# arkworks-rs/gemini

Measured on AMD Instinct MI355X. Metric: BLS12-381 G1 MSM throughput, higher is better.
Workload: dtype u32x12 Montgomery Fq (381-bit integer), u32x8 Fr; 1 GPU; 2^20 G1 MSM per GPU (BASELINE configs[1]: 2^20 G1 MSM on one MI355X); pairs_per_gpu=1048576

## Files before the change

### gemini_amd/capi.py

```python
from __future__ import annotations

import ctypes as C
import os

import numpy as np

_HERE = os.path.dirname(os.path.abspath(__file__))
LIB_PATH = os.environ.get("GM_LIB_PATH") or os.path.join(_HERE, "libgemini_hip.so")

GM_OK = 0
ERRORS = {-1: "GM_EINVAL", -2: "GM_ENOTINIT", -3: "GM_EHANDLE", -4: "GM_EHIP", -5: "GM_ENOMEM", -6: "GM_ESTATE"}

SYMBOLS = [
    "gm_init", "gm_shutdown", "gm_last_error", "gm_abi_version",
    "gm_g1_msm", "gm_g1_bases_register", "gm_g1_bases_free", "gm_g1_bases_len", "gm_g1_bases_download", "gm_g1_bases_precompute", "gm_set_auto_tables", "gm_g1_bases_table_info", "gm_pool_trim", "gm_g1_release_spare_tables", "gm_mem_stats", "gm_mem_reset_peak", "gm_runtime_info", "gm_snark_footprint", "gm_psnark_footprint", "gm_footprint_admit",
    "gm_g1_msm_h", "gm_g1_msm_v", "gm_g1_msm_v_batch", "gm_g1_msm_v_batch_partial", "gm_g1_msm_v_batch_at", "gm_g1_msm_d", "gm_g1_msm_d_partial", "gm_g1_sum",
    "gm_g1_msm_stream_new", "gm_g1_msm_stream_new_h", "gm_g1_msm_stream_add", "gm_g1_msm_stream_finalize", "gm_g1_msm_stream_free", "gm_host_alloc", "gm_host_free",
    "gm_g1_fixed_base_register", "gm_g1_srs_register", "gm_g1_srs_register_segments", "gm_set_msm_window", "gm_set_msm_table_min", "gm_set_msm_affine_levels", "gm_set_msm_split", "gm_set_msm_glv", "gm_prof_enable", "gm_prof_read", "gm_prof_read_clock",
    "gm_idx_register", "gm_idx_free", "gm_idx_len", "gm_idx_download", "gm_idx_extend_frequency", "gm_fr_gather", "gm_fr_alg_hash", "gm_fr_plookup_set", "gm_fr_add_scalar", "gm_fr_shift_monic",
    "gm_fr_acc_product", "gm_fr_tensor_range", "gm_fr_tensor_gather", "gm_fr_powers_gather", "gm_fr_alg_hash_from", "gm_fr_powers_range", "gm_fr_plookup_set_block", "gm_fr_shift_block", "gm_fr_product", "gm_fr_acc_product_block",
    "gm_sc_set_shard_rounds", "gm_sc_round_begin_many", "gm_psnark_shard_block", "gm_psnark_shard_level", "gm_psnark_shard_footprint", "gm_psnark_shard_key_new", "gm_psnark_index_sharded", "gm_psnark_new_time_sharded", "gm_snark_new_elastic_sharded",
    "gm_fr_vec_alloc", "gm_fr_vec_free", "gm_fr_vec_len", "gm_fr_vec_upload", "gm_fr_vec_download",
    "gm_fr_vec_fill", "gm_fr_vec_ptr", "gm_fr_vec_set_len",
    "gm_fr_reverse", "gm_fr_stride", "gm_fr_fold", "gm_fr_fold_chain", "gm_fr_powers", "gm_fr_tensor", "gm_fr_hadamard", "gm_fr_ip", "gm_fr_eval_le", "gm_fr_eval_le_batch",
    "gm_fr_lincomb", "gm_fr_scale_into", "gm_fr_scale_into_many", "gm_fr_add_at", "gm_fr_div_vanishing",
    "gm_spm_register", "gm_spm_free", "gm_spm_mul", "gm_spm_shape", "gm_snark_new_time", "gm_snark_new_elastic", "gm_psnark_new_time", "gm_psnark_new_elastic", "gm_psnark_preprocess", "gm_psnark_preprocess_free", "gm_psnark_index", "gm_spm_download",
    "gm_sc_new", "gm_sc_new_v", "gm_sc_new_borrow", "gm_sc_round", "gm_sc_round_begin", "gm_sc_round_end", "gm_sc_fold", "gm_sc_rounds", "gm_sc_final", "gm_sc_free",
    "gm_sc_set_shard", "gm_sc_lens", "gm_sc_download",
    "gm_sp_new", "gm_sp_new_v", "gm_sp_new_borrow", "gm_sp_round", "gm_sp_fold", "gm_sp_rounds", "gm_sp_final", "gm_sp_to_time", "gm_sp_free",
    "gm_sc_set_herring", "gm_hg1_new", "gm_hg1_round", "gm_hg1_fold", "gm_hg1_rounds", "gm_hg1_final", "gm_hg1_free",
    "gm_g2_msm", "gm_g2_bases_register", "gm_g2_bases_free", "gm_g2_bases_len", "gm_g2_bases_download", "gm_g2_msm_h", "gm_g2_msm_v", "gm_g2_msm_d", "gm_g2_sum",
    "gm_hg2_new", "gm_hg2_round", "gm_hg2_fold", "gm_hg2_rounds", "gm_hg2_final", "gm_hg2_free",
    "gm_pairing_multi", "gm_pairing_multi_h", "gm_gt_mul", "gm_gt_pow", "gm_gt_one", "gm_gt_final_exp",
# ... 121 lines not shown
```

### gemini_amd/csrc/capi.hip

```cpp
#include <cstring>
#include <vector>

#include "ctx.hpp"
#include "host_field.hpp"

namespace gm {

static thread_local char g_err[512] = "";
void set_error(const char* fmt, ...) {
  va_list ap;
  va_start(ap, fmt);
  vsnprintf(g_err, sizeof g_err, fmt, ap);
  va_end(ap);
}
int hip_fail(hipError_t e, const char* what, const char* file, int line) {
  set_error("HIP error %d (%s) in %s at %s:%d", (int)e, hipGetErrorString(e), what, file, line);
  return e == hipErrorOutOfMemory ? GM_ENOMEM : GM_EHIP;
}

MemStats& mem_stats() {
  static MemStats* m = new MemStats;
  return *m;
}
void MemStats::note_cached(ptrdiff_t delta) {
// ... 665 lines not shown
  GM_CTX();
  GM_CHECK(c == 0 || (c >= 2 && c <= 22), GM_EINVAL, "gm_set_msm_window: c = %d not in {0} u [2, 22]", c);
  C->msm_c_override = c;
  return GM_OK;
}

int gm_set_msm_glv(int on) {
  GM_CTX();
#ifndef GM_EXPERIMENTS
  GM_CHECK(on == 0, GM_EINVAL, "gm_set_msm_glv: the GLV experiment is not in this build (make EXTRA=-DGM_EXPERIMENTS; DESIGN.md section 8)");
#endif
  C->msm_glv = on != 0;
  return GM_OK;
}

int gm_set_msm_split(int on) {
  GM_CTX();
#ifndef GM_EXPERIMENTS
  GM_CHECK(on == 0, GM_EINVAL, "gm_set_msm_split: the window-group experiment is not in this build (make EXTRA=-DGM_EXPERIMENTS; DESIGN.md section 8)");
#endif
  C->msm_split = on != 0;
  return GM_OK;
}

int gm_set_msm_affine_levels(int levels) {
  GM_CTX();
  GM_CHECK(levels >= -1 && levels <= 8, GM_EINVAL, "gm_set_msm_affine_levels: %d not in [-1, 8]", levels);
#ifndef GM_EXPERIMENTS
  if (levels == -1) levels = 0;
  GM_CHECK(levels == 0, GM_EINVAL, "gm_set_msm_affine_levels: the affine-level experiment is not in this build (make EXTRA=-DGM_EXPERIMENTS; DESIGN.md section 8)");
// ... 1443 lines not shown
```

### gemini_amd/csrc/ctx.hpp

```cpp
#pragma once
#include <hip/hip_runtime.h>

#include <atomic>
#include <cstdarg>
#include <cstdint>
#include <cstdio>
#include <map>
#include <memory>
#include <mutex>
#include <string>
#include <unordered_map>
#include <vector>

#include "../../include/gemini_hip.h"

namespace gmh {
struct Fq12;
}

namespace gm {

void set_error(const char* fmt, ...);
int hip_fail(hipError_t e, const char* what, const char* file, int line);

// ... 148 lines not shown
};
struct G2Workspace {
  DevBuf buckets, part, red[2], longs;
  uint64_t* host_out = nullptr;
  size_t host_out_cap = 0;
};

struct PairingWorkspace {
  DevBuf part[2];
  uint64_t* host_out = nullptr;
  DevBuf seg_tab;
  uint64_t* host_seg = nullptr;
  size_t host_seg_cap = 0;
};
struct MsmWorkspace;
struct MsmPending {
  MsmWorkspace* ws = nullptr;
  int slot = 0;
  bool empty = true;
  int Wb = 0, c = 0, m = 0;
  uint32_t nbits = 0, wf[3] = {0, 0, 0};
  size_t plane_off[3] = {0, 0, 0};
  size_t plane_count = 0;
  int multi_levels = 0;
  int multi_W = 0;
};
struct MsmStreamSlot {
  uint8_t *raw = nullptr, *packed = nullptr, *scalars = nullptr;
  size_t raw_cap = 0, packed_cap = 0, scalars_cap = 0;
  hipEvent_t copied;
  bool have_ev = false;
  bool inflight = false;
  MsmPending P;
};
struct MsmStream {
  std::mutex mu;
  size_t chunk = 0, stride = 96;
  int mont = 0;
  uint64_t bases_handle = 0;
  int64_t base0 = 0, next_base = 0, step = 1;
// ... 89 lines not shown
  hipStream_t part_tail[2 + MSM_SMALL_LANES] = {};
  hipEvent_t start_ev;
  bool have_start_ev = false;
  DevBuf fr_scratch;
  uint64_t* host_small = nullptr;
  uint8_t* sc_desc_host = nullptr;
  uint8_t* sc_desc_dev = nullptr;
  hipEvent_t sc_desc_copied[SC_DESC_SLOTS] = {};
  unsigned sc_desc_next = 0;
  uint64_t* host_batch = nullptr;
  size_t host_batch_cap = 0;
  int msm_c_override = 0;
  int msm_glv = 0;
  int msm_split = 0;
  int msm_affine_levels = 0;
  size_t msm_table_min = (size_t)1 << 17;
  int zero_copy = 3;
  std::atomic<int> msm_busy{0};
  bool auto_tables = true;
  size_t auto_tables_max = 0;
  int cu_count = 256;
};

Context* context();
struct MemStats {
  std::mutex mu;
  std::unordered_map<void*, size_t> sizes;
  size_t live = 0, peak_live = 0;
  size_t cached = 0;
  size_t peak_in_use = 0;
// ... 122 lines not shown
```

### gemini_amd/csrc/msm.hip

```cpp
#include <algorithm>
#include <atomic>
#include <chrono>
#include <condition_variable>
#include <cstdlib>
#include <cstring>
#include <functional>
#include <sched.h>
#include <cstdio>
#include <thread>
#include <vector>

#include "ctx.hpp"
#include "g1.cuh"
#include "host_field.hpp"

namespace gm {

constexpr uint32_t KEY_INV = 0xffffffffu;
constexpr int XYZZ_BYTES = 192;
constexpr int AFF_BYTES = 96;

struct DigitIter {
  uint32_t s[8];
  uint32_t carry;
// ... 298 lines not shown
    const bool live = e[w] != ~0ull;
    const uint32_t g = (uint32_t)(e[w] >> 32) >> sg.FB;
    const uint32_t r = wave_atomic_inc(cnt, live ? g : KEY_INV);
    if (live) buf[lst[g] + r] = e[w];
  }
  __syncthreads();
  for (uint32_t j = tid; j < m; j += 1024) {
    const uint64_t v = buf[j];
    const uint32_t g = (uint32_t)(v >> 32) >> sg.FB;
    tmp[base[g] + (j - lst[g])] = v;
  }
}

__global__ __launch_bounds__(1024) void k_sort1_scan(const uint32_t* __restrict__ gcount, uint32_t G,
                                                     uint32_t* __restrict__ goff, uint32_t* __restrict__ gcursor,
                                                     uint32_t* __restrict__ blkoff) {
  __shared__ uint32_t a[1024], b[1024];
  const uint32_t tid = threadIdx.x;
  const uint32_t per = (G + 1023u) / 1024u;
  uint32_t v[4], nb[4], sa = 0, sb = 0;
  for (uint32_t k = 0; k < per; k++) {
    const uint32_t g = tid * per + k;
    v[k] = g < G ? gcount[g] : 0u;
    nb[k] = (v[k] + SORT_CH - 1u) / SORT_CH;
    sa += v[k];
    sb += nb[k];
  }
  a[tid] = sa;
  b[tid] = sb;
  __syncthreads();
  for (uint32_t d = 1; d < 1024; d <<= 1) {
// ... 5 lines not shown
  }
  uint32_t ra = a[tid] - sa, rb = b[tid] - sb;
  for (uint32_t k = 0; k < per; k++) {
    const uint32_t g = tid * per + k;
    if (g < G) {
      goff[g] = ra;
      gcursor[g] = ra;
      blkoff[g] = rb;
    }
    ra += v[k];
    rb += nb[k];
  }
  if (tid == 1023) {
    goff[G] = a[1023];
    blkoff[G] = b[1023];
  }
}

template <bool SCATTER>
__global__ __launch_bounds__(256) void k_sort2(const uint64_t* __restrict__ tmp, const uint32_t* __restrict__ goff,
                                               const uint32_t* __restrict__ blkoff, SortGeom sg,
                                               uint32_t* __restrict__ counts_or_cursor, uint64_t* __restrict__ entries) {
  __shared__ uint32_t cnt[SORT_FMAX];
  __shared__ uint32_t base[SCATTER ? SORT_FMAX : 1];
  __shared__ uint32_t s_g;
  const uint32_t nf = 1u << sg.FB;
  if (blockIdx.x >= blkoff[sg.G]) return;
  if (threadIdx.x == 0) {
    uint32_t lo = 0, hi = sg.G;
    while (hi - lo > 1) {
// ... 100 lines not shown
  __syncthreads();
  for (uint32_t f = tid; f < nf; f += 1024) cnt[f] = 0;
  __syncthreads();
#pragma unroll
  for (uint32_t k = 0; k < PER; k++) {
    const uint32_t i = tid + k * 1024;
    const uint32_t f = (uint32_t)(e[k] >> 32) & mask;
    const uint32_t r = wave_atomic_inc(cnt, i < m ? f : KEY_INV);
    if (i < m) buf[lst[f] + r] = e[k];
  }
  __syncthreads();
  for (uint32_t i = tid; i < m; i += 1024) {
    const uint64_t v = buf[i];
    const uint32_t f = (uint32_t)(v >> 32) & mask;
    entries[base[f] + (i - lst[f])] = v;
  }
}

constexpr uint32_t SCAN_PER_THREAD = 16;
constexpr uint32_t SCAN_PER_BLOCK = 256 * SCAN_PER_THREAD;

GM_DEV uint32_t block_exclusive_scan_256(uint32_t v, uint32_t* lds , uint32_t* total) {
  const uint32_t tid = threadIdx.x;
  lds[tid] = v;
  __syncthreads();
  for (uint32_t d = 1; d < 256; d <<= 1) {
    uint32_t x = tid >= d ? lds[tid - d] : 0;
    __syncthreads();
    lds[tid] += x;
    __syncthreads();
// ... 523 lines not shown
  uint32_t n_out;
  uint32_t per_win;
  uint32_t win_stride;
  uint32_t n_lo, s_hi, s_lo, s_e, len;
  uint32_t nb;
  uint32_t lpo_shift;
  int out_canonical;
  const uint32_t* in_cnt;
};
struct GroupSumJobs {
  GroupSumArgs j[3];
  uint32_t blk_end[3];
  const uint32_t* err_src;
  uint32_t* err_dst;
  const unsigned long long* clk_src;
};

__global__ __launch_bounds__(256) void k_group_sum(GroupSumJobs J) {
  if (J.err_dst && blockIdx.x == 0 && threadIdx.x == 0) {
    *J.err_dst = *J.err_src;
    if (J.clk_src) {
      unsigned long long* d = reinterpret_cast<unsigned long long*>(J.err_dst + 2);
      d[0] = J.clk_src[0];
      d[1] = J.clk_src[1];
    }
  }
  const int job = blockIdx.x < J.blk_end[0] ? 0 : (blockIdx.x < J.blk_end[1] ? 1 : 2);
  const GroupSumArgs& a = J.j[job];
  const uint32_t blk0 = job == 0 ? 0u : J.blk_end[job - 1];
  const uint8_t* __restrict__ in = a.in;
  uint8_t* __restrict__ out = a.out;
  const uint32_t gt = (blockIdx.x - blk0) * blockDim.x + threadIdx.x;
  const uint32_t lpo = 1u << a.lpo_shift;
  const uint32_t o = gt >> a.lpo_shift, q = gt & (lpo - 1u);
  Acc30 acc;
// ... 628 lines not shown
  }
  if (batch_trace)
    fprintf(stderr, "[gm msm batch] %zu calls: %.3f ms, of which enqueueing %.3f ms, final drains %.3f ms\n", k,
            std::chrono::duration<double, std::milli>(std::chrono::steady_clock::now() - t_batch0).count(), enqueue_s * 1e3,
            std::chrono::duration<double, std::milli>(std::chrono::steady_clock::now() - t_enqueued).count());
  return GM_OK;
}

static int msm_enqueue(Context* C, MsmWorkspace& ws, MsmStreams sts, const Bases* bases, int64_t first, int64_t step, const void* d_scalars,
                       int mont, size_t n, int slot, MsmPending* P, int part, int nparts, const MsmMulti* multi) {
  hipStream_t st = sts.sort;
  const size_t nbases = bases->n;
  P->ws = &ws;
  P->slot = slot;
  P->multi_levels = 0;
  if (multi) {
    GM_CHECK(multi->levels >= 1 && multi->levels <= MULTI_MAX_LEVELS && nparts == 1, GM_EINVAL, "msm: %d fused calls (1 .. %d)", multi->levels, MULTI_MAX_LEVELS);
    GM_CHECK(nbases <= ((size_t)1 << 30), GM_EINVAL, "msm: a key of %zu points is too long for a fused pass (2^30)", nbases);
    n = 0;
    for (int l = 0; l < multi->levels; l++) {
      GM_CHECK(multi->n[l] >= 1 && multi->n[l] <= (multi->block ? MSM_MULTI_BLOCK_MAX_N : MSM_MULTI_MAX_N), GM_EINVAL, "msm: a fused call of %zu pairs", multi->n[l]);
      const int64_t lo = multi->start[l], hi = multi->start[l] + step * (int64_t)(multi->n[l] - 1);
      GM_CHECK(lo >= 0 && hi >= 0 && (size_t)lo < nbases && (size_t)hi < nbases, GM_EINVAL, "msm: base range [%lld .. %lld] outside registered bases (len %zu)",
               (long long)lo, (long long)hi, nbases);
      n += multi->n[l];
    }
    first = 0;
  }
  P->empty = n == 0;
  if (n == 0) return GM_OK;
// ... 78 lines not shown
  uint64_t Nacc = N;
  for (int l = 0; l < levels; l++) Nacc = Nacc / 2 + 2 * nbuckets + 2;

  static const int L_env = getenv("GM_MSM_L") ? atoi(getenv("GM_MSM_L")) : 0;
  const uint64_t Nacc_all = nparts > 1 ? Nall : Nacc;
  const uint64_t lanes0 = Nacc_all >= ((uint64_t)1 << 24) ? 262144 : 131072;
  static const uint64_t L_cap = getenv("GM_MSM_LCAP") ? (uint64_t)atoi(getenv("GM_MSM_LCAP")) : 256;
  uint32_t L = (uint32_t)std::min<uint64_t>(L_cap, std::max<uint64_t>(4, (Nacc_all + lanes0 - 1) / lanes0));
  if (L_env > 0) L = (uint32_t)L_env;
  L = (L + 1u) & ~1u;
  const uint64_t T0 = (Nacc + L - 1) / L;
  const uint64_t T0pad = (T0 + 255) / 256 * 256;
  const uint64_t E1 = 2 * T0pad;

  int rc;
  const size_t counts_words = (nbuckets + 2 + SORT_GMAX + 1 + 63) / 64 * 64;
  if ((rc = ws.counts.ensure(counts_words * 4))) return rc;
  if ((rc = ws.offsets.ensure((nbuckets + 1) * 4))) return rc;
  if ((rc = ws.cursor.ensure((nbuckets + 1) * 4))) return rc;
  if ((rc = ws.misc.ensure((nbuckets / SCAN_PER_BLOCK + 2) * 4))) return rc;
  if ((rc = ws.entries.ensure(N * 8))) return rc;
  if ((rc = ws.buckets.ensure(nbuckets * bucket_bytes))) return rc;
  if ((rc = ws.pk[0].ensure(E1 * 4))) return rc;
  if ((rc = ws.pp[0].ensure(E1 * bucket_bytes))) return rc;
  const uint64_t E2 = 2 * ((E1 + 127) / 128);
  if ((rc = ws.pk[1].ensure(E2 * 4))) return rc;
  if ((rc = ws.pp[1].ensure(E2 * bucket_bytes))) return rc;

  const uint32_t* sc = reinterpret_cast<const uint32_t*>(d_scalars);
  GM_HIP(hipMemsetAsync(ws.counts.p, 0, counts_words * 4, st));
  uint32_t* d_err = ws.counts.as<uint32_t>() + nbuckets + 1;
  const bool bucket_counts_valid = levels == 0;
  if (!bucket_counts_valid) GM_HIP(hipMemsetAsync(ws.buckets.p, 0, nbuckets * bucket_bytes, st));
  const uint32_t dblocks = (uint32_t)((n + 255) / 256);
  Profiler& pf = C->prof;
  auto run_scan = [&]() {
    const uint32_t nb = (uint32_t)((nbuckets + SCAN_PER_BLOCK - 1) / SCAN_PER_BLOCK);
    hipLaunchKernelGGL(k_scan_block_sums, dim3(nb), dim3(256), 0, st, ws.counts.as<uint32_t>(), (uint32_t)nbuckets,
                       ws.misc.as<uint32_t>());
    hipLaunchKernelGGL(k_scan_top, dim3(1), dim3(1024), 0, st, ws.misc.as<uint32_t>(), nb,
                       ws.offsets.as<uint32_t>() + nbuckets);
    hipLaunchKernelGGL(k_scan_apply, dim3(nb), dim3(256), 0, st, ws.counts.as<uint32_t>(), (uint32_t)nbuckets,
                       ws.misc.as<uint32_t>(), ws.offsets.as<uint32_t>(), ws.cursor.as<uint32_t>());
  };
  static const bool sort_atomic_env = getenv("GM_MSM_SORT") && !strcmp(getenv("GM_MSM_SORT"), "atomic");
  static const bool sort_flat_env = !(getenv("GM_MSM_SORT") && !strcmp(getenv("GM_MSM_SORT"), "blocks"));
// ... 83 lines not shown
    sg.B = B;
    sg.shared = use_table ? 1 : 0;
    sg.FB = std::min<uint32_t>((uint32_t)(c - 1), 10u);
    if (multi_block) sg.FB = std::min<uint32_t>((uint32_t)(c - 1), std::max<uint32_t>(sg.FB, 11u));
    while ((nbuckets >> sg.FB) > SORT_GMAX && (1u << sg.FB) < SORT_FMAX) sg.FB++;
    sg.G = (uint32_t)(nbuckets >> sg.FB);
    GM_CHECK(sg.G <= SORT_GMAX, GM_EINVAL, "msm: %u coarse sort bins exceed %u (window %d too wide for this sort)", sg.G, SORT_GMAX, c);
    if ((rc = ws.tmp_entries.ensure(N * 8))) return rc;
    if ((rc = ws.sortmeta.ensure((size_t)(3 * (sg.G + 1)) * 4))) return rc;
    uint32_t* gcount = ws.counts.as<uint32_t>() + nbuckets + 2;
    uint32_t* goff = ws.sortmeta.as<uint32_t>();
    uint32_t* gcursor = goff + (sg.G + 1);
    uint32_t* blkoff = gcursor + (sg.G + 1);
    const uint32_t b1 = (uint32_t)((n + SORT_TS - 1) / SORT_TS);
    const uint32_t b2 = (uint32_t)(N / SORT_CH + sg.G + 1);
    pf.begin(part, PROF_DIGITS, st);
    hipLaunchKernelGGL(k_sort1<false>, dim3(b1), dim3(256), 0, st, sc, (uint32_t)n, mont, sg, lg, gcount, (uint64_t*)nullptr, d_err);
    hipLaunchKernelGGL(k_sort1_scan, dim3(1), dim3(1024), 0, st, gcount, sg.G, goff, gcursor, blkoff);
    const size_t stage1_lds = (size_t)SORT_TS * sg.Wg * (use_glv ? 2 : 1) * 8 + (size_t)3 * sg.G * 4 + 1024 * 4;
    static const bool sort1_staged_env = !(getenv("GM_MSM_SORT1") && !strcmp(getenv("GM_MSM_SORT1"), "direct"));
    if (sort1_staged_env && sg.Wg * (use_glv ? 2 : 1) <= SORT1_STAGE_WMAX && stage1_lds <= 160 * 1024) {
      static bool attr_set = false;
      if (!attr_set) {
        GM_HIP(hipFuncSetAttribute(reinterpret_cast<const void*>(k_sort1_staged), hipFuncAttributeMaxDynamicSharedMemorySize, 160 * 1024));
        attr_set = true;
      }
      hipLaunchKernelGGL(k_sort1_staged, dim3(b1), dim3(1024), stage1_lds, st, sc, (uint32_t)n, mont, sg, lg, gcursor, ws.tmp_entries.as<uint64_t>());
    } else {
      hipLaunchKernelGGL(k_sort1<true>, dim3(b1), dim3(256), 0, st, sc, (uint32_t)n, mont, sg, lg, gcursor, ws.tmp_entries.as<uint64_t>(), d_err);
    }
    pf.end(part, PROF_DIGITS, st);
    pf.begin(part, PROF_SCATTER, st);
    hipLaunchKernelGGL(k_sort2<false>, dim3(b2), dim3(256), 0, st, ws.tmp_entries.as<uint64_t>(), goff, blkoff, sg,
                       ws.counts.as<uint32_t>(), (uint64_t*)nullptr);
    run_scan();
    static const bool sort_staged = !(getenv("GM_MSM_SORT2") && !strcmp(getenv("GM_MSM_SORT2"), "direct"));
    if (sort_staged && (1u << sg.FB) <= SORT_STAGE_FMAX)
      hipLaunchKernelGGL(k_sort2_staged, dim3(b2), dim3(1024), 0, st, ws.tmp_entries.as<uint64_t>(), goff, blkoff, sg,
                         ws.cursor.as<uint32_t>(), ws.entries.as<uint64_t>());
    else
      hipLaunchKernelGGL(k_sort2<true>, dim3(b2), dim3(256), 0, st, ws.tmp_entries.as<uint64_t>(), goff, blkoff, sg,
                         ws.cursor.as<uint32_t>(), ws.entries.as<uint64_t>());
    pf.end(part, PROF_SCATTER, st);
  }
  const uint64_t* acc_entries = ws.entries.as<uint64_t>();
  const uint32_t* acc_total = ws.offsets.as<uint32_t>() + nbuckets;
  const uint8_t* acc_bases = d_bases;
  long long acc_first = (long long)first, acc_step = multi ? 1ll : (long long)step, acc_tab = tab_stride;
#ifdef GM_EXPERIMENTS
#define GM_MSM_LEVELS_HOST 1
#include "msm_levels.inc"
#undef GM_MSM_LEVELS_HOST
#else
  GM_CHECK(levels == 0, GM_EINVAL, "msm: affine tree levels are an experiment of round 2; rebuild with -DGM_EXPERIMENTS (DESIGN.md section 8)");
#endif
  if (!ws.have_done_ev) {
    for (int e = 0; e < MSM_SLOTS; e++) GM_HIP(hipEventCreateWithFlags(&ws.done_ev[e], hipEventDisableTiming));
// ... 85 lines not shown
    GroupSumArgs g{};
    g.in = in; g.out = out; g.mode = GS_PLANE; g.out_canonical = 1;
    g.in_cnt = in == bucket_in ? bucket_cnt : nullptr;
    g.per_win = nb + 1; g.n_out = (uint32_t)Wb * g.per_win; g.win_stride = 1u << nb; g.nb = nb;
    g.lpo_shift = lpo_for(nb ? (1u << (nb - 1)) : 1u, g.n_out);
    return g;
  };
  uint8_t* planes = nullptr;
  size_t plane_count = 0;
  auto launch = [&](std::initializer_list<GroupSumArgs> jobs, bool last = false) {
    GroupSumJobs J{};
    if (last) {
      J.err_src = d_err;
      J.err_dst = reinterpret_cast<uint32_t*>(planes + plane_count * XYZZ_BYTES);
      J.clk_src = ws.clk.as<unsigned long long>();
    }
    uint32_t tot = 0;
    int k = 0;
    for (const GroupSumArgs& g : jobs) {
      J.j[k] = g;
      tot += (uint32_t)((((uint64_t)g.n_out << g.lpo_shift) + 255) / 256);
      J.blk_end[k] = tot;
      k++;
    }
    for (; k < 3; k++) J.blk_end[k] = tot;
    hipLaunchKernelGGL(k_group_sum, dim3(tot), dim3(256), 0, st, J);
  };
  size_t plane_off[3];
  for (int k = 0; k < m; k++) {
    plane_off[k] = plane_count;
// ... 186 lines not shown
};

static void horner_pool_prewake() { HornerPool::get().prewake(); }
static void horner_pool_run(int n, const std::function<void(int)>& fn) { HornerPool::get().run(n, fn); }

static int msm_finish_parts(Context* C, const MsmPending* parts, int nparts, bool normalize, uint64_t out_jac[18], bool use_pool, uint64_t* const* multi_out) {
  gmh::G1 result = gmh::G1::identity();
  int rc = GM_OK;
  for (int p = nparts - 1; p >= 0; p--) {
    const MsmPending& P = parts[p];
    if (P.empty) continue;
    MsmWorkspace& ws = *P.ws;
    if (P.Wb > 1 && use_pool) HornerPool::get().prewake();
    GM_HIP(hipEventSynchronize(ws.done_ev[P.slot]));
    const uint64_t* hp = ws.host_planes[P.slot];
    if ((uint32_t)hp[P.plane_count * 24] != 0) {
      set_error("msm: a scalar passed as a canonical integer is >= 2^255 (not the BigInt image of an Fr element)");
      rc = GM_EINVAL;
      continue;
    }
    if (rc) continue;
    auto plane_at = [&](int w, int field, uint32_t j) {
      return gmh::xyzz_to_jac_dev(hp + (P.plane_off[field] + (size_t)w * (P.wf[field] + 1) + j) * 24);
    };
    std::vector<gmh::G1> S((size_t)P.Wb);
    auto window_sum = [&](int w) {
      gmh::G1 s = gmh::G1::identity();
      int field = P.m - 1;
      uint32_t jj = P.wf[field];
      for (int j = (int)P.nbits - 1; j >= 0; j--) {
// ... 93 lines not shown
    sg.FB = std::min<uint32_t>((uint32_t)(c - 1), 10u);
    while ((nbuckets >> sg.FB) > SORT_GMAX && (1u << sg.FB) < SORT_FMAX) sg.FB++;
    sg.G = (uint32_t)(nbuckets >> sg.FB);
    GM_CHECK(sg.G <= SORT_GMAX, GM_EINVAL, "msm sort: %u coarse sort bins exceed %u (window %d too wide for this sort)", sg.G, SORT_GMAX, c);
    if ((rc = ws.tmp_entries.ensure(N * 8))) return rc;
    if ((rc = ws.sortmeta.ensure((size_t)(3 * (sg.G + 1)) * 4))) return rc;
    LevelGeom lg{};
    uint32_t* gcount = ws.counts.as<uint32_t>() + nbuckets + 2;
    uint32_t* goff = ws.sortmeta.as<uint32_t>();
    uint32_t* gcursor = goff + (sg.G + 1);
    uint32_t* blkoff = gcursor + (sg.G + 1);
    const uint32_t b1 = (uint32_t)((n + SORT_TS - 1) / SORT_TS);
    const uint32_t b2 = (uint32_t)(N / SORT_CH + sg.G + 1);
    const uint32_t nb = (uint32_t)((nbuckets + SCAN_PER_BLOCK - 1) / SCAN_PER_BLOCK);
    hipLaunchKernelGGL(k_sort1<false>, dim3(b1), dim3(256), 0, st, sc, (uint32_t)n, mont, sg, lg, gcount, (uint64_t*)nullptr, d_err);
    hipLaunchKernelGGL(k_sort1_scan, dim3(1), dim3(1024), 0, st, gcount, sg.G, goff, gcursor, blkoff);
    hipLaunchKernelGGL(k_sort1<true>, dim3(b1), dim3(256), 0, st, sc, (uint32_t)n, mont, sg, lg, gcursor, ws.tmp_entries.as<uint64_t>(), d_err);
    hipLaunchKernelGGL(k_sort2<false>, dim3(b2), dim3(256), 0, st, ws.tmp_entries.as<uint64_t>(), goff, blkoff, sg, ws.counts.as<uint32_t>(),
                       (uint64_t*)nullptr);
    hipLaunchKernelGGL(k_scan_block_sums, dim3(nb), dim3(256), 0, st, ws.counts.as<uint32_t>(), (uint32_t)nbuckets, ws.misc.as<uint32_t>());
    hipLaunchKernelGGL(k_scan_top, dim3(1), dim3(1024), 0, st, ws.misc.as<uint32_t>(), nb, ws.offsets.as<uint32_t>() + nbuckets);
    hipLaunchKernelGGL(k_scan_apply, dim3(nb), dim3(256), 0, st, ws.counts.as<uint32_t>(), (uint32_t)nbuckets, ws.misc.as<uint32_t>(),
                       ws.offsets.as<uint32_t>(), ws.cursor.as<uint32_t>());
    hipLaunchKernelGGL(k_sort2<true>, dim3(b2), dim3(256), 0, st, ws.tmp_entries.as<uint64_t>(), goff, blkoff, sg, ws.cursor.as<uint32_t>(),
                       ws.entries.as<uint64_t>());
  }
  GM_HIP(hipGetLastError());
  out->entries = ws.entries.as<uint64_t>();
  out->offsets = ws.offsets.as<uint32_t>();
  out->err = d_err;
  out->W = W;
// ... 363 lines not shown
```

### include/gemini_hip.h

```cpp
#ifndef GEMINI_HIP_H
#define GEMINI_HIP_H

#include <stddef.h>
#include <stdint.h>

#ifdef __cplusplus
extern "C" {
#endif

#define GM_OK 0
#define GM_EINVAL (-1)
#define GM_ENOTINIT (-2)
#define GM_EHANDLE (-3)
#define GM_EHIP (-4)
#define GM_ENOMEM (-5)
#define GM_ESTATE (-6)

int gm_init(int device);
void gm_shutdown(void);
const char* gm_last_error(void);
int gm_abi_version(void);

int gm_g1_msm(const void* bases, size_t base_stride, const uint64_t* scalars, size_t n, uint64_t out_jac[18]);

// ... 38 lines not shown
int gm_g1_msm_stream_new_h(uint64_t bases_handle, size_t offset, int reversed, size_t chunk_pairs, int scalars_mont, uint64_t* stream);
int gm_g1_msm_stream_add(uint64_t stream, const void* bases_host, const void* scalars_host, size_t n);
int gm_g1_msm_stream_finalize(uint64_t stream, uint64_t out_jac[18], size_t* pairs_or_null);
int gm_g1_msm_stream_free(uint64_t stream);
int gm_host_alloc(size_t bytes, void** p);
int gm_host_free(void* p);

int gm_g1_fixed_base_register(const uint64_t base_affine[12], const uint64_t* scalars, size_t n, uint64_t* handle);
int gm_g1_srs_register(const uint64_t base_affine[12], const uint64_t tau[4], size_t n, uint64_t* handle);
int gm_g1_srs_register_segments(const uint64_t base_affine[12], const uint64_t tau[4], const size_t* starts, const size_t* counts, size_t nseg,
                                uint64_t* handle);

int gm_set_msm_window(int c);
int gm_set_msm_table_min(size_t n);
int gm_set_msm_glv(int on);
int gm_set_msm_split(int on);
int gm_set_msm_affine_levels(int levels);

#define GM_PROF_NSTAGES 8
int gm_prof_enable(int on);
int gm_prof_read(double* ms_out, uint64_t* count_out, int n);
int gm_prof_read_clock(double* acc0_mhz);

int gm_fr_vec_alloc(size_t n, uint64_t* handle);
int gm_fr_vec_free(uint64_t handle);
int gm_fr_vec_len(uint64_t handle, size_t* n);
int gm_fr_vec_upload(uint64_t handle, size_t offset, const uint64_t* mont, size_t n);
int gm_fr_vec_download(uint64_t handle, size_t offset, uint64_t* mont, size_t n);
int gm_fr_vec_fill(uint64_t handle, const uint64_t value_mont[4]);
int gm_fr_vec_ptr(uint64_t handle, void** dptr);
// ... 361 lines not shown
```

Before: 349.3 Mscalar/s.

## Add compact 32-bit staged sort with per-group LDS bucket sort for MSM

Result: faster. 360.0 Mscalar/s (median of 6 runs) (+3.1%).

```diff
diff --git a/gemini_amd/capi.py b/gemini_amd/capi.py
--- a/gemini_amd/capi.py
+++ b/gemini_amd/capi.py
@@ -16,7 +16,7 @@
     "gm_g1_msm", "gm_g1_bases_register", "gm_g1_bases_free", "gm_g1_bases_len", "gm_g1_bases_download", "gm_g1_bases_precompute", "gm_set_auto_tables", "gm_g1_bases_table_info", "gm_pool_trim", "gm_g1_release_spare_tables", "gm_mem_stats", "gm_mem_reset_peak", "gm_runtime_info", "gm_snark_footprint", "gm_psnark_footprint", "gm_footprint_admit",
     "gm_g1_msm_h", "gm_g1_msm_v", "gm_g1_msm_v_batch", "gm_g1_msm_v_batch_partial", "gm_g1_msm_v_batch_at", "gm_g1_msm_d", "gm_g1_msm_d_partial", "gm_g1_sum",
     "gm_g1_msm_stream_new", "gm_g1_msm_stream_new_h", "gm_g1_msm_stream_add", "gm_g1_msm_stream_finalize", "gm_g1_msm_stream_free", "gm_host_alloc", "gm_host_free",
-    "gm_g1_fixed_base_register", "gm_g1_srs_register", "gm_g1_srs_register_segments", "gm_set_msm_window", "gm_set_msm_table_min", "gm_set_msm_affine_levels", "gm_set_msm_split", "gm_set_msm_glv", "gm_prof_enable", "gm_prof_read", "gm_prof_read_clock",
+    "gm_g1_fixed_base_register", "gm_g1_srs_register", "gm_g1_srs_register_segments", "gm_set_msm_window", "gm_set_msm_table_min", "gm_set_msm_affine_levels", "gm_set_msm_split", "gm_set_msm_glv", "gm_set_msm_sort_group", "gm_debug_msm_sort_path", "gm_prof_enable", "gm_prof_read", "gm_prof_read_clock",
     "gm_idx_register", "gm_idx_free", "gm_idx_len", "gm_idx_download", "gm_idx_extend_frequency", "gm_fr_gather", "gm_fr_alg_hash", "gm_fr_plookup_set", "gm_fr_add_scalar", "gm_fr_shift_monic",
     "gm_fr_acc_product", "gm_fr_tensor_range", "gm_fr_tensor_gather", "gm_fr_powers_gather", "gm_fr_alg_hash_from", "gm_fr_powers_range", "gm_fr_plookup_set_block", "gm_fr_shift_block", "gm_fr_product", "gm_fr_acc_product_block",
     "gm_sc_set_shard_rounds", "gm_sc_round_begin_many", "gm_psnark_shard_block", "gm_psnark_shard_level", "gm_psnark_shard_footprint", "gm_psnark_shard_key_new", "gm_psnark_index_sharded", "gm_psnark_new_time_sharded", "gm_snark_new_elastic_sharded",
diff --git a/gemini_amd/csrc/capi.hip b/gemini_amd/csrc/capi.hip
--- a/gemini_amd/csrc/capi.hip
+++ b/gemini_amd/csrc/capi.hip
@@ -703,6 +703,25 @@
   return GM_OK;
 }
 
+int gm_set_msm_sort_group(int mode, size_t cap) {
+  GM_CTX();
+  GM_CHECK(mode == 0 || mode == 1, GM_EINVAL, "gm_set_msm_sort_group: mode = %d not in {0, 1}", mode);
+  GM_CHECK(cap == 0 || (cap >= MSM_SORT_GROUP_CAP_MIN && cap <= MSM_SORT_GROUP_CAP_MAX), GM_EINVAL,
+           "gm_set_msm_sort_group: a block stages %zu .. %zu entries in its LDS (0 = the most), not %zu", MSM_SORT_GROUP_CAP_MIN, MSM_SORT_GROUP_CAP_MAX, cap);
+  std::lock_guard<std::recursive_mutex> lk(C->msm_mu);
+  C->msm_sort_group = mode;
+  C->msm_sort_group_cap = cap;
+  return GM_OK;
+}
+
+int gm_debug_msm_sort_path(int* out) {
+  GM_CTX();
+  GM_CHECK(out != nullptr, GM_EINVAL, "gm_debug_msm_sort_path: null output");
+  std::lock_guard<std::recursive_mutex> lk(C->msm_mu);
+  *out = C->msm_sort_path_last;
+  return GM_OK;
+}
+
 int gm_set_msm_split(int on) {
   GM_CTX();
 #ifndef GM_EXPERIMENTS
diff --git a/gemini_amd/csrc/ctx.hpp b/gemini_amd/csrc/ctx.hpp
--- a/gemini_amd/csrc/ctx.hpp
+++ b/gemini_amd/csrc/ctx.hpp
@@ -186,6 +186,8 @@
   size_t host_seg_cap = 0;
 };
 struct MsmWorkspace;
+constexpr size_t MSM_SORT_GROUP_CAP_MAX = (160 * 1024 - 3 * 1024 * 4 - 64) / 4;
+constexpr size_t MSM_SORT_GROUP_CAP_MIN = 1024;
 struct MsmPending {
   MsmWorkspace* ws = nullptr;
   int slot = 0;
@@ -196,6 +198,7 @@
   size_t plane_count = 0;
   int multi_levels = 0;
   int multi_W = 0;
+  bool sort_compact = false;
 };
 struct MsmStreamSlot {
   uint8_t *raw = nullptr, *packed = nullptr, *scalars = nullptr;
@@ -315,6 +318,9 @@
   int msm_glv = 0;
   int msm_split = 0;
   int msm_affine_levels = 0;
+  int msm_sort_group = 1;
+  size_t msm_sort_group_cap = 0;
+  int msm_sort_path_last = 0;
   size_t msm_table_min = (size_t)1 << 17;
   int zero_copy = 3;
   std::atomic<int> msm_busy{0};
diff --git a/gemini_amd/csrc/msm.hip b/gemini_amd/csrc/msm.hip
--- a/gemini_amd/csrc/msm.hip
+++ b/gemini_amd/csrc/msm.hip
@@ -336,7 +336,7 @@
 
 __global__ __launch_bounds__(1024) void k_sort1_scan(const uint32_t* __restrict__ gcount, uint32_t G,
                                                      uint32_t* __restrict__ goff, uint32_t* __restrict__ gcursor,
-                                                     uint32_t* __restrict__ blkoff) {
+                                                     uint32_t* __restrict__ blkoff, uint32_t* __restrict__ total_out) {
   __shared__ uint32_t a[1024], b[1024];
   const uint32_t tid = threadIdx.x;
   const uint32_t per = (G + 1023u) / 1024u;
@@ -372,6 +372,7 @@
   if (tid == 1023) {
     goff[G] = a[1023];
     blkoff[G] = b[1023];
+    if (total_out) *total_out = a[1023];
   }
 }
 
@@ -502,6 +503,216 @@
     const uint64_t v = buf[i];
     const uint32_t f = (uint32_t)(v >> 32) & mask;
     entries[base[f] + (i - lst[f])] = v;
+  }
+}
+
+GM_DEV uint32_t sort_entry_expand_hi(uint32_t v, uint32_t g, uint32_t FB) { return (g << FB) | (v >> (32u - FB)); }
+GM_DEV uint64_t sort_entry_expand(uint32_t v, uint32_t g, uint32_t FB) {
+  const uint32_t ib = 31u - FB;
+  return ((uint64_t)sort_entry_expand_hi(v, g, FB) << 32) | (uint64_t)(((v >> ib) & 1u) << 31) | (uint64_t)(v & ((1u << ib) - 1u));
+}
+
+__global__ __launch_bounds__(1024) void k_sort1_staged_c(const uint32_t* __restrict__ scalars, uint32_t n, int mont, SortGeom sg,
+                                                         uint32_t* __restrict__ gcursor, uint32_t* __restrict__ tmp) {
+  extern __shared__ __attribute__((aligned(16))) uint8_t smem[];
+  uint32_t* buf = reinterpret_cast<uint32_t*>(smem);
+  uint32_t* cnt = buf + (size_t)SORT_TS * sg.Wg;
+  uint32_t* base = cnt + sg.G;
+  uint32_t* lst = base + sg.G;
+  uint32_t* scan = lst + sg.G;
+  const uint32_t tid = threadIdx.x;
+  for (uint32_t g = tid; g < sg.G; g += 1024) cnt[g] = 0;
+  __syncthreads();
+  const uint32_t i = blockIdx.x * SORT_TS + tid;
+  const bool active = i < n;
+  uint32_t ks[SORT1_STAGE_WMAX];
+  {
+    DigitIter it;
+    it.init(scalars + 8 * (size_t)(active ? i : 0), active, mont);
+#pragma unroll
+    for (int j = 0; j < SORT1_STAGE_WMAX; j++) {
+      uint32_t k = ~0u;
+      if (j < sg.Wg) {
+        const int32_t d = j == sg.W - 1 ? it.last(sg.c) : it.next(sg.c);
+        if (active && d != 0) k = ((uint32_t)j * sg.B + ((uint32_t)(d < 0 ? -d : d) - 1u)) | (d < 0 ? 0x80000000u : 0u);
+      }
+      ks[j] = k;
+      wave_atomic_inc(cnt, k != ~0u ? (k & 0x7fffffffu) >> sg.FB : KEY_INV);
+    }
+  }
+  __syncthreads();
+  const uint32_t per = (sg.G + 1023u) / 1024u;
+  uint32_t s = 0;
+  for (uint32_t k = 0; k < per; k++) {
+    const uint32_t g = tid * per + k;
+    if (g < sg.G) {
+      const uint32_t c = cnt[g];
+      base[g] = c ? atomicAdd(gcursor + g, c) : 0u;
+      s += c;
+    }
+  }
+  scan[tid] = s;
+  __syncthreads();
+  for (uint32_t d = 1; d < 1024; d <<= 1) {
+    const uint32_t x = tid >= d ? scan[tid - d] : 0;
+    __syncthreads();
+    scan[tid] += x;
+    __syncthreads();
+  }
+  uint32_t run = scan[tid] - s;
+  for (uint32_t k = 0; k < per; k++) {
+    const uint32_t g = tid * per + k;
+    if (g < sg.G) {
+      lst[g] = run;
+      run += cnt[g];
+    }
+  }
+  __syncthreads();
+  for (uint32_t g = tid; g < sg.G; g += 1024) cnt[g] = 0;
+  __syncthreads();
+  const uint32_t ib = 31u - sg.FB, fmask = (1u << sg.FB) - 1u;
+#pragma unroll
+  for (int j = 0; j < SORT1_STAGE_WMAX; j++) {
+    const uint32_t k = ks[j];
+    const bool live = k != ~0u;
+    const uint32_t key = k & 0x7fffffffu, g = key >> sg.FB;
+    const uint32_t r = wave_atomic_inc(cnt, live ? g : KEY_INV);
+    if (live) buf[lst[g] + r] = ((key & fmask) << (ib + 1u)) | ((k >> 31) << ib) | i;
+  }
+  __syncthreads();
+  const uint32_t hw = tid >> 5, hl = tid & 31u;
+  for (uint32_t k = 0; k * 32u < sg.G; k++) {
+    const uint32_t g = k * 32u + ((hw + k) & 31u);
+    if (g >= sg.G) continue;
+    const uint32_t c = cnt[g], l0 = lst[g], b0 = base[g];
+    for (uint32_t o = hl; o < c; o += 32u) tmp[b0 + o] = buf[l0 + o];
+  }
+}
+
+GM_DEV uint32_t block_inclusive_scan_1024(uint32_t v, uint32_t* wsum ) {
+  const uint32_t lane = threadIdx.x & 63u, wv = threadIdx.x >> 6;
+#pragma unroll
+  for (uint32_t d = 1; d < 64; d <<= 1) {
+    const uint32_t x = __shfl_up(v, d);
+    if (lane >= d) v += x;
+  }
+  __syncthreads();
+  if (lane == 63) wsum[wv] = v;
+  __syncthreads();
+  uint32_t add = 0;
+  for (uint32_t k = 0; k < wv; k++) add += wsum[k];
+  return v + add;
+}
+
+constexpr uint32_t SORT2G_QPT = 10;
+static_assert(SORT2G_QPT * 4096 >= MSM_SORT_GROUP_CAP_MAX + 3, "k_sort2_group: a chunk must fit the registers of its block");
+template <uint32_t QPT>
+struct Sort2gChunk {
+  uint32_t v[4 * QPT];
+  uint32_t off, nq, mc;
+  GM_DEV void load(const uint32_t* __restrict__ tmp, uint32_t s0, uint32_t mc_) {
+    mc = mc_;
+    off = s0 & 3u;
+    nq = (off + mc + 3u) >> 2;
+    const uint4* t4 = reinterpret_cast<const uint4*>(tmp) + (s0 >> 2);
+#pragma unroll
+    for (uint32_t kq = 0; kq < QPT; kq++) {
+      const uint32_t q = kq * 1024 + threadIdx.x;
+      uint4 x = make_uint4(0, 0, 0, 0);
+      if (q < nq) x = t4[q];
+      v[4 * kq] = x.x;
+      v[4 * kq + 1] = x.y;
+      v[4 * kq + 2] = x.z;
+      v[4 * kq + 3] = x.w;
+    }
+  }
+  GM_DEV uint32_t at(uint32_t kq, uint32_t t) const { return 4u * (kq * 1024 + threadIdx.x) + t - off; }
+  GM_DEV void count(uint32_t* cnt, uint32_t fsh) const {
+#pragma unroll
+    for (uint32_t kq = 0; kq < QPT; kq++) {
+      if (kq * 1024 < nq) {
+#pragma unroll
+        for (uint32_t t = 0; t < 4; t++) wave_atomic_inc(cnt, at(kq, t) < mc ? v[4 * kq + t] >> fsh : KEY_INV);
+      }
+    }
+  }
+};
+__global__ __launch_bounds__(1024) void k_sort2_group(const uint32_t* __restrict__ tmp, const uint32_t* __restrict__ goff, SortGeom sg, uint32_t cap,
+                                                      uint32_t* __restrict__ counts, uint32_t* __restrict__ offsets, uint64_t* __restrict__ entries,
+                                                      uint32_t* __restrict__ chunked) {
+  extern __shared__ __attribute__((aligned(16))) uint8_t smem[];
+  uint32_t* ccnt = reinterpret_cast<uint32_t*>(smem);
+  uint32_t* clst = ccnt + 1024;
+  uint32_t* glst = clst + 1024;
+  uint32_t* wsum = glst + 1024;
+  uint32_t* buf = wsum + 16;
+  const uint32_t tid = threadIdx.x, g = blockIdx.x;
+  const uint32_t nf = 1u << sg.FB, fsh = 32u - sg.FB, b0 = g << sg.FB;
+  const uint32_t lo = goff[g], m = goff[g + 1] - lo;
+  if (m == 0) {
+    if (tid < nf) offsets[b0 + tid] = lo;
+    return;
+  }
+  const bool single = m <= cap;
+  if (!single) {
+    glst[tid] = 0;
+    __syncthreads();
+    constexpr uint32_t CQ = 4;
+    for (uint32_t c0 = 0; c0 < m; c0 += CQ * 4096 - 3) {
+      Sort2gChunk<CQ> ch;
+      ch.load(tmp, lo + c0, min(CQ * 4096 - 3, m - c0));
+      ch.count(glst, fsh);
+    }
+    __syncthreads();
+    const uint32_t c = glst[tid];
+    const uint32_t ex = block_inclusive_scan_1024(c, wsum) - c;
+    if (tid < nf) {
+      counts[b0 + tid] = c;
+      offsets[b0 + tid] = lo + ex;
+    }
+    glst[tid] = ex;
+    if (tid == 0) *chunked = 1u;
+  }
+  for (uint32_t c0 = 0; c0 < m; c0 += cap) {
+    const uint32_t mc = min(cap, m - c0);
+    ccnt[tid] = 0;
+    __syncthreads();
+    Sort2gChunk<SORT2G_QPT> ch;
+    ch.load(tmp, lo + c0, mc);
+    ch.count(ccnt, fsh);
+    __syncthreads();
+    const uint32_t c = ccnt[tid];
+    const uint32_t ex = block_inclusive_scan_1024(c, wsum) - c;
+    clst[tid] = ex;
+    if (single && tid < nf) {
+      counts[b0 + tid] = c;
+      offsets[b0 + tid] = lo + ex;
+    }
+    ccnt[tid] = 0;
+    __syncthreads();
+#pragma unroll
+    for (uint32_t kq = 0; kq < SORT2G_QPT; kq++) {
+      if (kq * 1024 < ch.nq) {
+#pragma unroll
+        for (uint32_t t = 0; t < 4; t++) {
+          const bool live = ch.at(kq, t) < mc;
+          const uint32_t x = ch.v[4 * kq + t], f = x >> fsh;
+          const uint32_t r = wave_atomic_inc(ccnt, live ? f : KEY_INV);
+          if (live) buf[clst[f] + r] = x;
+        }
+      }
+    }
+    __syncthreads();
+    if (single) {
+      for (uint32_t j = tid; j < mc; j += 1024) entries[lo + j] = sort_entry_expand(buf[j], g, sg.FB);
+    } else {
+      for (uint32_t j = tid; j < mc; j += 1024) {
+        const uint32_t x = buf[j], f = x >> fsh;
+        entries[lo + glst[f] + (j - clst[f])] = sort_entry_expand(x, g, sg.FB);
+      }
+      __syncthreads();
+      glst[tid] += ccnt[tid];
+    }
   }
 }
 
@@ -1055,11 +1266,13 @@
   const uint32_t* err_src;
   uint32_t* err_dst;
   const unsigned long long* clk_src;
+  const uint32_t* chunked_src;
 };
 
 __global__ __launch_bounds__(256) void k_group_sum(GroupSumJobs J) {
   if (J.err_dst && blockIdx.x == 0 && threadIdx.x == 0) {
     *J.err_dst = *J.err_src;
+    J.err_dst[1] = J.chunked_src ? *J.chunked_src : 0u;
     if (J.clk_src) {
       unsigned long long* d = reinterpret_cast<unsigned long long*>(J.err_dst + 2);
       d[0] = J.clk_src[0];
@@ -1718,6 +1931,7 @@
   P->ws = &ws;
   P->slot = slot;
   P->multi_levels = 0;
+  P->sort_compact = false;
   if (multi) {
     GM_CHECK(multi->levels >= 1 && multi->levels <= MULTI_MAX_LEVELS && nparts == 1, GM_EINVAL, "msm: %d fused calls (1 .. %d)", multi->levels, MULTI_MAX_LEVELS);
     GM_CHECK(nbases <= ((size_t)1 << 30), GM_EINVAL, "msm: a key of %zu points is too long for a fused pass (2^30)", nbases);
@@ -1826,7 +2040,7 @@
   const uint64_t E1 = 2 * T0pad;
 
   int rc;
-  const size_t counts_words = (nbuckets + 2 + SORT_GMAX + 1 + 63) / 64 * 64;
+  const size_t counts_words = (nbuckets + 2 + SORT_GMAX + 2 + 63) / 64 * 64;
   if ((rc = ws.counts.ensure(counts_words * 4))) return rc;
   if ((rc = ws.offsets.ensure((nbuckets + 1) * 4))) return rc;
   if ((rc = ws.cursor.ensure((nbuckets + 1) * 4))) return rc;
@@ -1842,6 +2056,7 @@
   const uint32_t* sc = reinterpret_cast<const uint32_t*>(d_scalars);
   GM_HIP(hipMemsetAsync(ws.counts.p, 0, counts_words * 4, st));
   uint32_t* d_err = ws.counts.as<uint32_t>() + nbuckets + 1;
+  uint32_t* d_chunked = ws.counts.as<uint32_t>() + nbuckets + 2 + SORT_GMAX + 1;
   const bool bucket_counts_valid = levels == 0;
   if (!bucket_counts_valid) GM_HIP(hipMemsetAsync(ws.buckets.p, 0, nbuckets * bucket_bytes, st));
   const uint32_t dblocks = (uint32_t)((n + 255) / 256);
@@ -1955,12 +2170,28 @@
     uint32_t* blkoff = gcursor + (sg.G + 1);
     const uint32_t b1 = (uint32_t)((n + SORT_TS - 1) / SORT_TS);
     const uint32_t b2 = (uint32_t)(N / SORT_CH + sg.G + 1);
+    static const bool sort1_staged_env = !(getenv("GM_MSM_SORT1") && !strcmp(getenv("GM_MSM_SORT1"), "direct"));
+    static const bool sort_staged = !(getenv("GM_MSM_SORT2") && !strcmp(getenv("GM_MSM_SORT2"), "direct"));
+    const size_t stage1c_lds = (size_t)SORT_TS * sg.Wg * 4 + (size_t)3 * sg.G * 4 + 1024 * 4;
+    const bool sort_compact = C->msm_sort_group == 1 && !use_table && !use_glv && !multi && nparts == 1 && N > ((uint64_t)1 << 21) &&
+                              sg.FB <= 10 && ceil_log2_sz(n) + (int)sg.FB + 1 <= 32 && sort1_staged_env && sort_staged &&
+                              sg.Wg <= SORT1_STAGE_WMAX && stage1c_lds <= 160 * 1024;
+    P->sort_compact = sort_compact;
+    uint32_t* tmp32 = ws.tmp_entries.as<uint32_t>();
     pf.begin(part, PROF_DIGITS, st);
     hipLaunchKernelGGL(k_sort1<false>, dim3(b1), dim3(256), 0, st, sc, (uint32_t)n, mont, sg, lg, gcount, (uint64_t*)nullptr, d_err);
-    hipLaunchKernelGGL(k_sort1_scan, dim3(1), dim3(1024), 0, st, gcount, sg.G, goff, gcursor, blkoff);
+    hipLaunchKernelGGL(k_sort1_scan, dim3(1), dim3(1024), 0, st, gcount, sg.G, goff, gcursor, blkoff,
+                       sort_compact ? ws.offsets.as<uint32_t>() + nbuckets : (uint32_t*)nullptr);
     const size_t stage1_lds = (size_t)SORT_TS * sg.Wg * (use_glv ? 2 : 1) * 8 + (size_t)3 * sg.G * 4 + 1024 * 4;
-    static const bool sort1_staged_env = !(getenv("GM_MSM_SORT1") && !strcmp(getenv("GM_MSM_SORT1"), "direct"));
-    if (sort1_staged_env && sg.Wg * (use_glv ? 2 : 1) <= SORT1_STAGE_WMAX && stage1_lds <= 160 * 1024) {
+    if (sort_compact) {
+      static bool attr_set = false;
+      if (!attr_set) {
+        GM_HIP(hipFuncSetAttribute(reinterpret_cast<const void*>(k_sort1_staged_c), hipFuncAttributeMaxDynamicSharedMemorySize, 160 * 1024));
+        GM_HIP(hipFuncSetAttribute(reinterpret_cast<const void*>(k_sort2_group), hipFuncAttributeMaxDynamicSharedMemorySize, 160 * 1024));
+        attr_set = true;
+      }
+      hipLaunchKernelGGL(k_sort1_staged_c, dim3(b1), dim3(1024), stage1c_lds, st, sc, (uint32_t)n, mont, sg, gcursor, tmp32);
+    } else if (sort1_staged_env && sg.Wg * (use_glv ? 2 : 1) <= SORT1_STAGE_WMAX && stage1_lds <= 160 * 1024) {
       static bool attr_set = false;
       if (!attr_set) {
         GM_HIP(hipFuncSetAttribute(reinterpret_cast<const void*>(k_sort1_staged), hipFuncAttributeMaxDynamicSharedMemorySize, 160 * 1024));
@@ -1972,16 +2203,21 @@
     }
     pf.end(part, PROF_DIGITS, st);
     pf.begin(part, PROF_SCATTER, st);
-    hipLaunchKernelGGL(k_sort2<false>, dim3(b2), dim3(256), 0, st, ws.tmp_entries.as<uint64_t>(), goff, blkoff, sg,
-                       ws.counts.as<uint32_t>(), (uint64_t*)nullptr);
-    run_scan();
-    static const bool sort_staged = !(getenv("GM_MSM_SORT2") && !strcmp(getenv("GM_MSM_SORT2"), "direct"));
-    if (sort_staged && (1u << sg.FB) <= SORT_STAGE_FMAX)
-      hipLaunchKernelGGL(k_sort2_staged, dim3(b2), dim3(1024), 0, st, ws.tmp_entries.as<uint64_t>(), goff, blkoff, sg,
-                         ws.cursor.as<uint32_t>(), ws.entries.as<uint64_t>());
-    else
-      hipLaunchKernelGGL(k_sort2<true>, dim3(b2), dim3(256), 0, st, ws.tmp_entries.as<uint64_t>(), goff, blkoff, sg,
-                         ws.cursor.as<uint32_t>(), ws.entries.as<uint64_t>());
+    if (sort_compact) {
+      const uint32_t cap = (uint32_t)(C->msm_sort_group_cap ? C->msm_sort_group_cap : MSM_SORT_GROUP_CAP_MAX);
+      hipLaunchKernelGGL(k_sort2_group, dim3(sg.G), dim3(1024), (size_t)(3 * 1024 + 16 + cap) * 4, st, tmp32, goff, sg, cap, ws.counts.as<uint32_t>(),
+                         ws.offsets.as<uint32_t>(), ws.entries.as<uint64_t>(), d_chunked);
+    } else {
+      hipLaunchKernelGGL(k_sort2<false>, dim3(b2), dim3(256), 0, st, ws.tmp_entries.as<uint64_t>(), goff, blkoff, sg,
+                         ws.counts.as<uint32_t>(), (uint64_t*)nullptr);
+      run_scan();
+      if (sort_staged && (1u << sg.FB) <= SORT_STAGE_FMAX)
+        hipLaunchKernelGGL(k_sort2_staged, dim3(b2), dim3(1024), 0, st, ws.tmp_entries.as<uint64_t>(), goff, blkoff, sg,
+                           ws.cursor.as<uint32_t>(), ws.entries.as<uint64_t>());
+      else
+        hipLaunchKernelGGL(k_sort2<true>, dim3(b2), dim3(256), 0, st, ws.tmp_entries.as<uint64_t>(), goff, blkoff, sg,
+                           ws.cursor.as<uint32_t>(), ws.entries.as<uint64_t>());
+    }
     pf.end(part, PROF_SCATTER, st);
   }
   const uint64_t* acc_entries = ws.entries.as<uint64_t>();
@@ -2097,6 +2333,7 @@
       J.err_src = d_err;
       J.err_dst = reinterpret_cast<uint32_t*>(planes + plane_count * XYZZ_BYTES);
       J.clk_src = ws.clk.as<unsigned long long>();
+      J.chunked_src = d_chunked;
     }
     uint32_t tot = 0;
     int k = 0;
@@ -2313,6 +2550,7 @@
     if (P.Wb > 1 && use_pool) HornerPool::get().prewake();
     GM_HIP(hipEventSynchronize(ws.done_ev[P.slot]));
     const uint64_t* hp = ws.host_planes[P.slot];
+    C->msm_sort_path_last = P.sort_compact ? 1 + (int)((hp[P.plane_count * 24] >> 32) != 0) : 0;
     if ((uint32_t)hp[P.plane_count * 24] != 0) {
       set_error("msm: a scalar passed as a canonical integer is >= 2^255 (not the BigInt image of an Fr element)");
       rc = GM_EINVAL;
@@ -2436,7 +2674,7 @@
     const uint32_t b2 = (uint32_t)(N / SORT_CH + sg.G + 1);
     const uint32_t nb = (uint32_t)((nbuckets + SCAN_PER_BLOCK - 1) / SCAN_PER_BLOCK);
     hipLaunchKernelGGL(k_sort1<false>, dim3(b1), dim3(256), 0, st, sc, (uint32_t)n, mont, sg, lg, gcount, (uint64_t*)nullptr, d_err);
-    hipLaunchKernelGGL(k_sort1_scan, dim3(1), dim3(1024), 0, st, gcount, sg.G, goff, gcursor, blkoff);
+    hipLaunchKernelGGL(k_sort1_scan, dim3(1), dim3(1024), 0, st, gcount, sg.G, goff, gcursor, blkoff, (uint32_t*)nullptr);
     hipLaunchKernelGGL(k_sort1<true>, dim3(b1), dim3(256), 0, st, sc, (uint32_t)n, mont, sg, lg, gcursor, ws.tmp_entries.as<uint64_t>(), d_err);
     hipLaunchKernelGGL(k_sort2<false>, dim3(b2), dim3(256), 0, st, ws.tmp_entries.as<uint64_t>(), goff, blkoff, sg, ws.counts.as<uint32_t>(),
                        (uint64_t*)nullptr);
diff --git a/include/gemini_hip.h b/include/gemini_hip.h
--- a/include/gemini_hip.h
+++ b/include/gemini_hip.h
@@ -76,6 +76,8 @@
 int gm_set_msm_window(int c);
 int gm_set_msm_table_min(size_t n);
 int gm_set_msm_glv(int on);
+int gm_set_msm_sort_group(int mode, size_t cap);
+int gm_debug_msm_sort_path(int* out);
 int gm_set_msm_split(int on);
 int gm_set_msm_affine_levels(int levels);
 
```
